# ultralytics/yolov3

Hardware: AMD Instinct MI355X
Metric: images/sec (640x640) inference+NMS (higher is better)
Workload: dtype f16; 1 GPU; yolov3 inference 640x640 batch=32/GPU fp16 nc=80 + NMS(conf 0.001, iou 0.6, multi_label, max_det 300) [BASELINE configs[1]]; global_batch=32, parallelism=replicas x1 (no data-path collective)

## Files before the change

### yolov3_amd/csrc/api.cpp

```cpp
#include <atomic>
#include <mutex>
#include <stdarg.h>
#include <stdio.h>
#include <stdlib.h>
#include <string.h>

#include "../../include/yolov3_hip.h"
#include "y3_knobs.h"

static thread_local char g_err[512] = "";

void y3_set_error(const char* fmt, ...) {
    va_list ap;
    va_start(ap, fmt);
    vsnprintf(g_err, sizeof(g_err), fmt, ap);
    va_end(ap);
}

extern "C" const char* y3_last_error(void) { return g_err; }
extern "C" int y3_abi_version(void) { return Y3_ABI_VERSION; }

namespace {
struct Knob {
    const char* name;
    long long def;
};
const Knob kKnobs[] = {
    {"conv", 0}, {"conv_ahead", 3}, {"bn_nt_bytes", 64ll << 20},
    {"wgrad", 0}, {"wgrad_xcd", 2}, {"dgrad_quad", 1}, {"spp_direct", 0}, {"wgrad_strip", 1}, {"conv_strip", 1},
    {"conv_v10", 1}, {"v10_mp", 0}, {"v10_blocks", 0}, {"v10_half", 2}, {"v10_ksplit", 1}, {"v10_slices", 0},
    {"v10_group", 1}, {"tile_xcd", 1}, {"conv_1x1s", 1}, {"wgrad_patch", 1}, {"wgrad_blocks", 512}, {"nms_sort", 1},
    {"decode_tile", 1},
};
constexpr int kCount = (int)(sizeof(kKnobs) / sizeof(kKnobs[0]));
static_assert(kCount == Y3K_COUNT, "kKnobs and y3_knob_id (y3_common.h) list the same knobs in the same order");
std::atomic<long long> g_val[kCount];
std::once_flag g_once;

int knob_index(const char* key) {
    for (int i = 0; i < kCount; ++i)
        if (key && !strcmp(key, kKnobs[i].name)) return i;
    return -1;
}
void load_defaults() {
    for (int i = 0; i < kCount; ++i) g_val[i].store(kKnobs[i].def, std::memory_order_relaxed);
    const char* e = getenv("Y3_TUNE");
    if (!e) return;
    char buf[512];
    strncpy(buf, e, sizeof(buf) - 1);
    buf[sizeof(buf) - 1] = 0;
    for (char* tok = strtok(buf, ",;"); tok; tok = strtok(nullptr, ",;")) {
        char* eq = strchr(tok, '=');
        if (!eq) continue;
        *eq = 0;
        const int i = knob_index(tok);
        if (i >= 0) g_val[i].store(atoll(eq + 1), std::memory_order_relaxed);
        else fprintf(stderr, "libyolov3_hip: Y3_TUNE names an unknown knob '%s'\n", tok);
    }
}
}

long long y3_knob(int id) {
    std::call_once(g_once, load_defaults);
    return (id >= 0 && id < kCount) ? g_val[id].load(std::memory_order_relaxed) : 0;
}
// ... 27 lines not shown
```

### yolov3_amd/csrc/detect_nms.hip

```cpp
#include "y3_common.h"

#include <rocprim/rocprim.hpp>

#include <atomic>

namespace {

template <typename T>
Y3_DEV float decode_one(float v, int o, int x, int y, float stride, float aw, float ah);

template <typename T>
__global__ __launch_bounds__(256) void decode_kernel(const T* __restrict__ head, int bs, int ny, int nx, int pitch, int na, int no, float aw0, float ah0,
                                                       float aw1, float ah1, float aw2, float ah2, float aw3, float ah3, float aw4, float ah4, float stride,
                                                       T* __restrict__ raw, T* __restrict__ z, long long row_offset, long long total_rows) {
    const int nch = na * no;
    const long long idx = (long long)blockIdx.x * 256 + threadIdx.x;
    const long long total = (long long)bs * ny * nx * nch;
    if (idx >= total) return;
    const int ch = (int)(idx % nch);
    long long t = idx / nch;
    const int x = (int)(t % nx);
    t /= nx;
    const int y = (int)(t % ny);
    const int b = (int)(t / ny);
// ... 185 lines not shown
            if (want_z) *(vec8*)((T*)job.z + (it.b * zimg + (L.row_offset + (long long)it.p0) * no) + off) = zv;
        }
    };
    const int step = gridDim.x;
    int item = blockIdx.x;
    Item ic = locate(item), i0, i1 = locate(item + step);
    uint4 v0 = load(ic), v1 = load(i1);
    ((uint4*)stage[0])[tid] = v0;
    __syncthreads();
    while (item < job.items) {
        i0 = locate(item + 2 * step);
        v0 = load(i0);
        compute(ic, stage[0], stage[1], v1);
        __syncthreads();
        ic = i1;
        if ((item += step) >= job.items) break;
        i1 = locate(item + 2 * step);
        v1 = load(i1);
        compute(ic, stage[1], stage[0], v0);
        __syncthreads();
        ic = i0;
        item += step;
    }
}

constexpr int IMG_BITS = 11, ORD_BITS = 21, CLS_BITS = 12, RANK_BITS = 15;
constexpr unsigned long long KEY_UNUSED = ~0ull;

struct NmsWs {
    int* row_count;
    int* row_off;
    unsigned* img_maxabs;
    unsigned* img_total;
    unsigned long long* key_a;
    unsigned long long* key_b;
    unsigned* val_a;
    unsigned* val_b;
    unsigned long long* key_c;
    unsigned* val_c;
    float4* cbox;
    float* cscore;
    int* ccls;
    float4* sbox;
    unsigned char* keep;
    void* tmp;
    size_t tmp_bytes;
    long long cap;
    int own_sort;
};

template <typename T> Y3_DEV bool gt_thr(float v, float thr_T) { return v > thr_T; }

Y3_DEV bool class_allowed(int c, const int* __restrict__ classes, int ncf) {
    if (ncf == 0) return true;
    bool ok = false;
    for (int i = 0; i < ncf; ++i) ok |= (classes[i] == c);
    return ok;
}

constexpr int NMS_ROW_BATCH = 8;
template <typename T, int MODE>
__global__ __launch_bounds__(256) void nms_candidates_kernel(const T* __restrict__ pred, int bs, int n_rows, int nc, float thr, int multi_label,
                                                               const int* __restrict__ classes, int ncf, NmsWs ws, int* __restrict__ status, int ord_shift) {
    const int lane = threadIdx.x & 63;
    const int chunks_per_img = (n_rows + 63) / 64;
    const long long wave_id = (long long)blockIdx.x * 4 + (threadIdx.x >> 6);
// ... 140 lines not shown
            cnt = ok ? 1 : 0;
            if (MODE == 1 && ok && lane == 0) {
                const long long g = off;
                if (g < ws.cap) {
                    const unsigned ord = (unsigned)((g - img_off0) >> ord_shift);
                    ws.cbox[g] = box;
                    ws.cscore[g] = best;
                    ws.ccls[g] = bi;
                    if (!ws.own_sort) {
                        ws.key_a[g] = ((unsigned long long)img << (32 + ORD_BITS)) | ((unsigned long long)(~__float_as_uint(best)) << ORD_BITS) |
                                      (unsigned long long)(ord & ((1u << ORD_BITS) - 1u));
                        ws.val_a[g] = (unsigned)g;
                    }
                } else {
                    status[0] = 1;
                }
            }
        }
        if (MODE == 1 && cnt > 0) {
            const float m4 = fmaxf(fmaxf(fabsf(box.x), fabsf(box.y)), fmaxf(fabsf(box.z), fabsf(box.w)));
            maxabs = (m4 == m4) ? fmaxf(maxabs, m4) : INFINITY;
        }
        if (lane == r) mycount = cnt;
    }
    if (MODE == 0) {
        if (myrow < n_rows) ws.row_count[(long long)img * n_rows + myrow] = mycount;
        if (ws.own_sort) {
            int t = mycount;
#pragma unroll
            for (int d = 32; d >= 1; d >>= 1) t += __shfl_xor(t, d);
            if (lane == 0 && t > 0) atomicAdd(&ws.img_total[img * 64 + (int)(wave_id & 63)], (unsigned)t);
        }
    } else {
        if (lane == 0 && maxabs > 0.0f) atomicMax(&ws.img_maxabs[img], __float_as_uint(maxabs));
    }
}

constexpr int SCAN_PER = 33, SCAN_CHUNK = 1024 * SCAN_PER;
__global__ __launch_bounds__(1024) void nms_scan_kernel(NmsWs ws, int bs, int n_rows) {
    __shared__ unsigned buf[SCAN_CHUNK];
    __shared__ unsigned wsum[16];
    const int img = blockIdx.x, tid = threadIdx.x, lane = tid & 63, wv = tid >> 6;
    auto block_sum_scan = [&](unsigned v, unsigned& excl, unsigned& total) {
        unsigned inc = v;
#pragma unroll
        for (int d = 1; d < 64; d <<= 1) {
            const unsigned o = __shfl_up(inc, d);
            if (lane >= d) inc += o;
        }
        __syncthreads();
        if (lane == 63) wsum[wv] = inc;
        __syncthreads();
        unsigned before = 0, all = 0;
#pragma unroll
        for (int w = 0; w < 16; ++w) {
            const unsigned t = wsum[w];
            if (w < wv) before += t;
            all += t;
        }
        excl = before + inc - v;
        total = all;
    };
    unsigned prev = 0;
    for (int j = tid; j < img * 64; j += 1024) prev += ws.img_total[j];
    unsigned e0, carry;
    block_sum_scan(prev, e0, carry);
    const int* __restrict__ cnt = ws.row_count + (long long)img * n_rows;
    int* __restrict__ off = ws.row_off + (long long)img * n_rows;
// ... 7 lines not shown
        for (int r = r0; r < r1; ++r) mine += buf[r];
        unsigned excl, total;
        block_sum_scan(mine, excl, total);
        unsigned run = carry + excl;
        for (int r = r0; r < r1; ++r) {
            const unsigned c = buf[r];
            buf[r] = run;
            run += c;
        }
        __syncthreads();
        for (int i = tid; i < n; i += 1024) off[c0 + i] = (int)buf[i];
        carry += total;
    }
    if (img == bs - 1 && tid == 0) ws.row_off[(long long)bs * n_rows] = (int)carry;
}

__global__ __launch_bounds__(256) void nms_rank_kernel(NmsWs ws, int bs, int n_rows, int max_nms, float max_wh, int agnostic, const unsigned long long* __restrict__ key1,
                                                        const unsigned* __restrict__ idx1, unsigned long long* __restrict__ key2, unsigned* __restrict__ val2,
                                                        int* __restrict__ status) {
    const long long i = (long long)blockIdx.x * 256 + threadIdx.x;
    if (i >= ws.cap) return;
    const long long total = ws.row_off[(long long)bs * n_rows];
    if (i == 0) status[1] = (int)(total > 0x7fffffffLL ? 0x7fffffff : total);
    unsigned long long k2 = KEY_UNUSED;
    ws.keep[i] = 0;
    if (i < total && key1[i] != KEY_UNUSED) {
        const int img = (int)(key1[i] >> (32 + ORD_BITS));
        const long long start = ws.row_off[(long long)img * n_rows];
        const long long rank = i - start;
        if (rank < max_nms) {
            const unsigned g = idx1[i];
            const int cls = ws.ccls[g];
            const float4 b = ws.cbox[g];
            const bool part = !agnostic && (__uint_as_float(ws.img_maxabs[img]) < max_wh * 0.5f);
            const float c = (float)cls * (agnostic ? 0.0f : max_wh);
            ws.sbox[i] = make_float4(b.x + c, b.y + c, b.z + c, b.w + c);
            const unsigned seg = part ? (unsigned)cls : 0u;
            k2 = ((unsigned long long)img << (CLS_BITS + RANK_BITS)) | ((unsigned long long)seg << RANK_BITS) | (unsigned long long)rank;
        }
    }
    key2[i] = k2;
    val2[i] = (unsigned)i;
}

constexpr int SORT_WAVES = 16, SORT_NB = 512;
struct SortLds {
    unsigned hist[SORT_WAVES * SORT_NB];
    unsigned tot[SORT_NB];
};
Y3_DEV unsigned ld_l2(const unsigned* p) { return __hip_atomic_load(p, __ATOMIC_RELAXED, __HIP_MEMORY_SCOPE_AGENT); }

template <typename Load, typename Digit, typename Put>
Y3_DEV void counting_pass(SortLds& L, const int cnt, const int bits, Load load, Digit digit, Put put) {
    const int tid = threadIdx.x, lane = tid & 63, wv = tid >> 6;
    const int nb = 1 << bits;
    for (int i = tid; i < SORT_WAVES * nb; i += SORT_WAVES * 64) L.hist[(i >> bits) * SORT_NB + (i & (nb - 1))] = 0u;
    __syncthreads();
    const int per = (((cnt + SORT_WAVES - 1) / SORT_WAVES) + 63) & ~63;
    const int lo = wv * per, hi = cnt < lo + per ? cnt : lo + per;
    for (int c0 = lo; c0 < hi; c0 += 256) {
        uint2 e[4];
#pragma unroll
        for (int u = 0; u < 4; ++u) {
            const int r = c0 + 64 * u + lane;
            e[u] = load(r < hi ? r : lo);
        }
#pragma unroll
        for (int u = 0; u < 4; ++u) {
            const int r = c0 + 64 * u + lane;
            if (r < hi) atomicAdd(&L.hist[wv * SORT_NB + digit(e[u].x)], 1u);
        }
    }
    __syncthreads();
    if (tid < nb) {
        unsigned run = 0;
#pragma unroll
        for (int w = 0; w < SORT_WAVES; ++w) {
            const unsigned t = L.hist[w * SORT_NB + tid];
            L.hist[w * SORT_NB + tid] = run;
            run += t;
        }
        L.tot[tid] = run;
    }
    __syncthreads();
    if (wv == 0) {
        unsigned v[SORT_NB / 64], sum = 0;
#pragma unroll
        for (int k = 0; k < SORT_NB / 64; ++k) {
            const int d = lane * (SORT_NB / 64) + k;
            v[k] = d < nb ? L.tot[d] : 0u;
            sum += v[k];
        }
        unsigned inc = sum;
#pragma unroll
        for (int d = 1; d < 64; d <<= 1) {
            const unsigned o = __shfl_up(inc, d);
            if (lane >= d) inc += o;
        }
        unsigned run = inc - sum;
#pragma unroll
        for (int k = 0; k < SORT_NB / 64; ++k) {
            const int d = lane * (SORT_NB / 64) + k;
            if (d < nb) L.tot[d] = run;
            run += v[k];
        }
    }
    __syncthreads();
    volatile unsigned* H = L.hist + wv * SORT_NB;
    const unsigned long long below = (1ull << lane) - 1ull;
    for (int c0 = lo; c0 < hi; c0 += 256) {
        uint2 e[4];
#pragma unroll
        for (int u = 0; u < 4; ++u) {
            const int r = c0 + 64 * u + lane;
            e[u] = load(r < hi ? r : lo);
        }
#pragma unroll
        for (int u = 0; u < 4; ++u) {
            if (c0 + 64 * u >= hi) break;
            const int r = c0 + 64 * u + lane;
            const bool valid = r < hi;
            const unsigned d = digit(e[u].x);
            unsigned long long peers = __ballot(valid);
            for (int b = 0; b < bits; ++b) {
                const bool bit = (d >> b) & 1u;
                const unsigned long long m = __ballot(valid && bit);
                peers &= bit ? m : ~m;
            }
            if (valid) {
                const unsigned base = H[d];
                put(L.tot[d] + base + (unsigned)__builtin_popcountll(peers & below), e[u].x, e[u].y);
                if ((peers >> lane) == 1ull) H[d] = base + (unsigned)__builtin_popcountll(peers);
            }
        }
    }
    __syncthreads();
}

__global__ __launch_bounds__(SORT_WAVES * 64) void nms_sort_kernel(NmsWs ws, int bs, int n_rows, int max_nms, float max_wh, int agnostic, int nseg, int sbit0, int sbits,
                                                                     int n_sp, int* __restrict__ status) {
    __shared__ SortLds L;
    const int img = blockIdx.x, tid = threadIdx.x;
    const long long total = ws.row_off[(long long)bs * n_rows];
    if (img == 0 && tid == 0) status[1] = (int)(total > 0x7fffffffLL ? 0x7fffffff : total);
    const long long start = ws.row_off[(long long)img * n_rows];
    long long cnt_ll = (long long)ws.row_off[(long long)(img + 1) * n_rows] - start;
    if (start + cnt_ll > ws.cap) cnt_ll = ws.cap - start > 0 ? ws.cap - start : 0;
    const int cnt = (int)cnt_ll;
    if (cnt <= 0) return;
    unsigned* const X0 = (unsigned*)ws.key_a + start, * const X1 = (unsigned*)ws.key_a + ws.cap + start;
    unsigned* const X2 = (unsigned*)ws.key_b + start, * const X3 = (unsigned*)ws.key_b + ws.cap + start;
    unsigned* const X4 = (unsigned*)ws.key_c + start, * const X5 = (unsigned*)ws.key_c + ws.cap + start;
    unsigned* const VA = ws.val_a + start, * const VB = ws.val_b + start, * const VC = ws.val_c + start;
    const float* __restrict__ score = ws.cscore + start;

    const unsigned dmask = (1u << sbits) - 1u;
    for (int p = 0; p < n_sp; ++p) {
        const int shift = sbit0 + p * sbits;
        const bool last = p == n_sp - 1;
        const unsigned* kin = p == 1 ? X0 : p == 2 ? X2 : X5;
        const unsigned* vin = p == 1 ? X1 : p == 2 ? X3 : VA;
        unsigned* kout = p == 0 ? X0 : p == 1 ? X2 : X5;
        unsigned* vout = last ? VB : p == 0 ? X1 : p == 1 ? X3 : VA;
        counting_pass(
            L, cnt, sbits,
            [&](int r) { return p == 0 ? make_uint2(~__float_as_uint(score[r]), (unsigned)(start + r)) : make_uint2(ld_l2(kin + r), ld_l2(vin + r)); },
            [&](unsigned k) { return (k >> shift) & dmask; },
            [&](unsigned pos, unsigned k, unsigned v) {
                if (!last) kout[pos] = k;
                vout[pos] = v;
            });
    }

    const int cntm = cnt < max_nms ? cnt : max_nms;
    const bool part = !agnostic && nseg > 1 && (__uint_as_float(ws.img_maxabs[img]) < max_wh * 0.5f);
    for (int r = tid; r < cntm; r += SORT_WAVES * 64) {
        const unsigned g = ld_l2(VB + r);
        const float4 b = ws.cbox[g];
        const float c = (float)ws.ccls[g] * (agnostic ? 0.0f : max_wh);
        ws.sbox[start + r] = make_float4(b.x + c, b.y + c, b.z + c, b.w + c);
        ws.keep[start + r] = 0;
        if (!part) { VC[r] = (unsigned)(start + r); X4[r] = 0u; }
    }
    if (!part) return;
    int cbits = 1;
    while ((1 << cbits) < nseg) ++cbits;
    auto seg_of = [&](int r) { return make_uint2((unsigned)ws.ccls[ld_l2(VB + r)], (unsigned)(start + r)); };
    if (cbits <= 9) {
        counting_pass(L, cntm, cbits, seg_of, [&](unsigned k) { return k; }, [&](unsigned pos, unsigned k, unsigned v) { X4[pos] = k; VC[pos] = v; });
    } else {
        counting_pass(L, cntm, 9, seg_of, [&](unsigned k) { return k & 511u; }, [&](unsigned pos, unsigned k, unsigned v) { X0[pos] = k; X1[pos] = v; });
        counting_pass(
            L, cntm, cbits - 9, [&](int r) { return make_uint2(ld_l2(X0 + r), ld_l2(X1 + r)); }, [&](unsigned k) { return k >> 9; },
            [&](unsigned pos, unsigned k, unsigned v) { X4[pos] = k; VC[pos] = v; });
    }
}

Y3_DEV long long lower_bound_u64(const unsigned long long* __restrict__ a, long long n, unsigned long long v) {
    long long lo = 0, hi = n;
    while (lo < hi) {
        const long long mid = (lo + hi) >> 1;
        if (a[mid] < v) lo = mid + 1; else hi = mid;
    }
    return lo;
}

Y3_DEV long long lower_bound_u32(const unsigned* __restrict__ a, long long n, unsigned v) {
    long long lo = 0, hi = n;
    while (lo < hi) {
        const long long mid = (lo + hi) >> 1;
        if (a[mid] < v) lo = mid + 1; else hi = mid;
    }
    return lo;
}

__global__ __launch_bounds__(256) void nms_greedy_kernel(NmsWs ws, int nseg, double iou_thr, int max_det, int max_nms, const unsigned long long* __restrict__ key2,
                                                          const unsigned* __restrict__ pos2, const unsigned* __restrict__ seg_sorted, int n_rows) {
    __shared__ unsigned removed[(1 << RANK_BITS) / 32];
    __shared__ float4 blk[64];
    __shared__ unsigned long long srow[64];
    __shared__ unsigned long long s_keepm;
    __shared__ int s_kept;
    const int img = blockIdx.x / nseg, seg = blockIdx.x % nseg;
    long long lo, hi;
    if (seg_sorted) {
        const long long start = ws.row_off[(long long)img * n_rows];
        long long cnt = (long long)ws.row_off[(long long)(img + 1) * n_rows] - start;
        if (start + cnt > ws.cap) cnt = ws.cap - start > 0 ? ws.cap - start : 0;
        if (cnt > max_nms) cnt = max_nms;
        lo = start + lower_bound_u32(seg_sorted + start, cnt, (unsigned)seg);
        hi = start + lower_bound_u32(seg_sorted + start, cnt, (unsigned)seg + 1u);
    } else {
        const unsigned long long kbase = ((unsigned long long)img << (CLS_BITS + RANK_BITS)) | ((unsigned long long)seg << RANK_BITS);
        lo = lower_bound_u64(key2, ws.cap, kbase);
        hi = lower_bound_u64(key2, ws.cap, kbase + (1ull << RANK_BITS));
    }
    const int n = (int)(hi - lo);
    if (n <= 0) return;
    const int tid = threadIdx.x, lane = tid & 63, wv = tid >> 6;
    for (int w = tid; w < 2 * ((n + 63) / 64); w += 256) removed[w] = 0u;
    if (tid == 0) s_kept = 0;
    const unsigned* __restrict__ pos = pos2 + lo;
    auto suppresses = [&](const float4 bi, const float iarea, const float4 bj) {
        const float xx1 = fmaxf(bi.x, bj.x), yy1 = fmaxf(bi.y, bj.y);
        const float xx2 = fminf(bi.z, bj.z), yy2 = fminf(bi.w, bj.w);
        float w = xx2 - xx1, h = yy2 - yy1;
        w = w > 0.0f ? w : 0.0f;
        h = h > 0.0f ? h : 0.0f;
        const float inter = w * h;
        const float jarea = (bj.z - bj.x) * (bj.w - bj.y);
        const float ovr = inter / (iarea + jarea - inter);
        return (double)ovr > iou_thr;
    };
    for (int base = 0; base < n; base += 64) {
        const int cnt = n - base < 64 ? n - base : 64;
        __syncthreads();
        const unsigned long long rem_in = (unsigned long long)removed[base >> 5] | ((unsigned long long)removed[(base >> 5) + 1] << 32);
        const unsigned long long valid = cnt == 64 ? ~0ull : ((1ull << cnt) - 1ull);
        if ((rem_in & valid) == valid) continue;
        if (tid < 64) {
            if (tid < cnt) blk[tid] = ws.sbox[pos[base + tid]];
            srow[tid] = 0ull;
// ... 12 lines not shown
        }
        __syncthreads();
        if (wv == 0) {
            const unsigned long long row = srow[lane];
            const int row_lo = (int)(unsigned)row, row_hi = (int)(unsigned)(row >> 32);
            unsigned long long rem = rem_in, keepm = 0ull;
            int kept = s_kept;
            for (int i = 0; i < cnt && kept < max_det; ++i) {
                if (!((rem >> i) & 1ull)) {
                    keepm |= 1ull << i;
                    ++kept;
                    rem |= (unsigned long long)(unsigned)__builtin_amdgcn_readlane(row_lo, i) | ((unsigned long long)(unsigned)__builtin_amdgcn_readlane(row_hi, i) << 32);
                }
            }
            if ((keepm >> lane) & 1ull) ws.keep[pos[base + lane]] = 1;
            if (lane == 0) { s_keepm = keepm; s_kept = kept; }
        }
        __syncthreads();
        const unsigned long long keepm = s_keepm;
        if (s_kept >= max_det) break;
        if (keepm)
            for (int j = base + 64 + tid; j < n; j += 256) {
                if (removed[j >> 5] & (1u << (j & 31))) continue;
                const float4 bj = ws.sbox[pos[j]];
                unsigned long long km = keepm;
                while (km) {
                    const int i = __builtin_ctzll(km);
                    km &= km - 1ull;
                    const float4 bi = blk[i];
                    if (suppresses(bi, (bi.z - bi.x) * (bi.w - bi.y), bj)) { atomicOr(&removed[j >> 5], 1u << (j & 31)); break; }
                }
            }
    }
}

__global__ __launch_bounds__(256) void nms_gather_kernel(NmsWs ws, int n_rows, int max_det, int max_nms, const unsigned* __restrict__ idx1,
                                                          float* __restrict__ out_rows, int* __restrict__ out_counts) {
    __shared__ int wave_cnt[4];
    __shared__ int s_base;
    const int img = blockIdx.x;
    const long long start = ws.row_off[(long long)img * n_rows];
    long long cnt = (long long)ws.row_off[(long long)(img + 1) * n_rows] - start;
    if (start + cnt > ws.cap) cnt = ws.cap - start > 0 ? ws.cap - start : 0;
    if (cnt > max_nms) cnt = max_nms;
    const int tid = threadIdx.x, lane = tid & 63, wv = tid >> 6;
    if (tid == 0) s_base = 0;
    __syncthreads();
    for (long long c0 = 0; c0 < cnt; c0 += 256) {
        const long long i = c0 + tid;
        const bool k = (i < cnt) && ws.keep[start + i];
        const unsigned long long m = __ballot(k);
        if (lane == 0) wave_cnt[wv] = __builtin_popcountll(m);
        __syncthreads();
        int before = s_base;
        for (int w = 0; w < wv; ++w) before += wave_cnt[w];
        const int slot = before + __builtin_popcountll(m & ((1ull << lane) - 1ull));
        if (k && slot < max_det) {
            const unsigned g = idx1[start + i];
            const float4 b = ws.cbox[g];
            float* o = out_rows + ((long long)img * max_det + slot) * 6;
            o[0] = b.x; o[1] = b.y; o[2] = b.z; o[3] = b.w;
            o[4] = ws.cscore[g];
            o[5] = (float)ws.ccls[g];
        }
        __syncthreads();
        if (tid == 0) s_base += wave_cnt[0] + wave_cnt[1] + wave_cnt[2] + wave_cnt[3];
        __syncthreads();
        if (s_base >= max_det) break;
    }
    if (tid == 0) out_counts[img] = s_base < max_det ? s_base : max_det;
}

size_t align_up(size_t v) { return (v + 255) & ~(size_t)255; }

long long worst_capacity(int bs, int n_rows, int nc, const y3_nms_params* p) {
    return (long long)bs * n_rows * ((p->multi_label && nc > 1) ? nc : 1);
}
long long default_capacity(int bs, int n_rows, int nc, const y3_nms_params* p) {
    const long long worst = worst_capacity(bs, n_rows, nc, p);
    long long cap = (long long)bs * 16384;
    if (cap > worst) cap = worst;
    if (cap < 1024) cap = 1024;
    return cap;
}

size_t temp_bytes(long long cap, size_t scan_n) {
    size_t a = 0, b = 0;
    (void)rocprim::radix_sort_pairs(nullptr, a, (unsigned long long*)nullptr, (unsigned long long*)nullptr, (unsigned*)nullptr, (unsigned*)nullptr, (size_t)cap, 0u,
                                    64u, (hipStream_t)0);
    (void)rocprim::exclusive_scan(nullptr, b, (int*)nullptr, (int*)nullptr, 0, scan_n + 1, rocprim::plus<int>(), (hipStream_t)0);
    return align_up(a > b ? a : b);
}

size_t carve(NmsWs& ws, unsigned char* base, int bs, long long cap, size_t scan_n) {
    size_t off = 0;
    auto take = [&](size_t bytes) {
        unsigned char* p = base ? base + off : nullptr;
        off += align_up(bytes);
        return p;
    };
    ws.cap = cap;
    ws.row_count = (int*)take((scan_n + 1) * sizeof(int));
    ws.row_off = (int*)take((scan_n + 1) * sizeof(int));
    ws.img_maxabs = (unsigned*)take((size_t)65 * bs * sizeof(unsigned));
    ws.img_total = ws.img_maxabs ? ws.img_maxabs + bs : nullptr;
    ws.key_a = (unsigned long long*)take((size_t)cap * 8);
    ws.key_b = (unsigned long long*)take((size_t)cap * 8);
    ws.key_c = (unsigned long long*)take((size_t)cap * 8);
    ws.val_a = (unsigned*)take((size_t)cap * 4);
    ws.val_b = (unsigned*)take((size_t)cap * 4);
    ws.val_c = (unsigned*)take((size_t)cap * 4);
    ws.cbox = (float4*)take((size_t)cap * 16);
    ws.cscore = (float*)take((size_t)cap * 4);
    ws.ccls = (int*)take((size_t)cap * 4);
    ws.sbox = (float4*)take((size_t)cap * 16);
    ws.keep = (unsigned char*)take((size_t)cap);
    ws.tmp_bytes = temp_bytes(cap, scan_n);
    ws.tmp = take(ws.tmp_bytes);
    return off;
}

template <typename T>
int run_nms(const void* pred, int bs, int n_rows, int nc, const y3_nms_params* p, const int* classes, float* out_rows, int* out_counts, int* out_status,
            long long capacity, void* workspace, size_t workspace_bytes, hipStream_t st) {
    const size_t scan_n = (size_t)bs * n_rows;
    long long cap = capacity > 0 ? capacity : default_capacity(bs, n_rows, nc, p);
    const long long worst = worst_capacity(bs, n_rows, nc, p);
    if (cap > worst) cap = worst;
    if (cap < 1024) cap = 1024;
    NmsWs ws;
    const size_t need = carve(ws, nullptr, bs, cap, scan_n);
    if (need > workspace_bytes) Y3_FAIL("y3_nms: workspace too small (%zu bytes given, %zu needed for capacity %lld)", workspace_bytes, need, cap);
    if (cap > 0x7ffffff0LL) Y3_FAIL("y3_nms: capacity too large");
    carve(ws, (unsigned char*)workspace, bs, cap, scan_n);

    const float thr = (float)(T)(p->conf_thres);
    const int multi = (p->multi_label && nc > 1) ? 1 : 0;
    const int ncf = classes ? p->n_classes_filter : 0;
    int ord_shift = 0;
    while ((((long long)n_rows * (multi ? nc : 1)) >> ord_shift) >= (1ll << ORD_BITS)) ++ord_shift;
    const bool one_seg = p->agnostic != 0;
    const int nseg = one_seg ? 1 : nc;

    Y3_HIP(hipMemsetAsync(out_status, 0, 2 * sizeof(int), st));
    Y3_HIP(hipMemsetAsync(ws.img_maxabs, 0, (size_t)65 * bs * sizeof(unsigned), st));
    ws.own_sort = y3_knob(Y3K_NMS_SORT) != 0 ? 1 : 0;
    if (!ws.own_sort) Y3_HIP(hipMemsetAsync(ws.key_a, 0xff, (size_t)cap * 8, st));
    Y3_HIP(hipMemsetAsync(ws.row_count + scan_n, 0, sizeof(int), st));

    const long long waves = (long long)bs * ((n_rows + 63) / 64);
    const unsigned cblocks = (unsigned)((waves + 3) / 4);
    hipLaunchKernelGGL((nms_candidates_kernel<T, 0>), dim3(cblocks), dim3(256), 0, st, (const T*)pred, bs, n_rows, nc, thr, multi, classes, ncf, ws, out_status, ord_shift);
    Y3_CHECK_LAUNCH();
    size_t tb = ws.tmp_bytes;
    if (ws.own_sort) {
        hipLaunchKernelGGL(nms_scan_kernel, dim3((unsigned)bs), dim3(1024), 0, st, ws, bs, n_rows);
        Y3_CHECK_LAUNCH();
    } else if (rocprim::exclusive_scan(ws.tmp, tb, ws.row_count, ws.row_off, 0, scan_n + 1, rocprim::plus<int>(), st) != hipSuccess) Y3_FAIL("y3_nms: scan failed");
    hipLaunchKernelGGL((nms_candidates_kernel<T, 1>), dim3(cblocks), dim3(256), 0, st, (const T*)pred, bs, n_rows, nc, thr, multi, classes, ncf, ws, out_status, ord_shift);
    Y3_CHECK_LAUNCH();
    if (ws.own_sort) {
        const bool narrow = sizeof(T) == 2;
        hipLaunchKernelGGL(nms_sort_kernel, dim3((unsigned)bs), dim3(SORT_WAVES * 64), 0, st, ws, bs, n_rows, p->max_nms, p->max_wh, p->agnostic, nseg, narrow ? 13 : 0,
                           narrow ? 9 : 8, narrow ? 2 : 4, out_status);
        Y3_CHECK_LAUNCH();
        hipLaunchKernelGGL(nms_greedy_kernel, dim3((unsigned)(bs * nseg)), dim3(256), 0, st, ws, nseg, p->iou_thres, p->max_det, p->max_nms,
                           (const unsigned long long*)nullptr, ws.val_c, (const unsigned*)ws.key_c, n_rows);
        Y3_CHECK_LAUNCH();
        hipLaunchKernelGGL(nms_gather_kernel, dim3((unsigned)bs), dim3(256), 0, st, ws, n_rows, p->max_det, p->max_nms, ws.val_b, out_rows, out_counts);
        Y3_CHECK_LAUNCH();
        return 0;
    }
    tb = ws.tmp_bytes;
    if (rocprim::radix_sort_pairs(ws.tmp, tb, ws.key_a, ws.key_b, ws.val_a, ws.val_b, (size_t)cap, 0u, 64u, st) != hipSuccess) Y3_FAIL("y3_nms: sort-1 failed");
    const unsigned rblocks = (unsigned)((cap + 255) / 256);
    hipLaunchKernelGGL(nms_rank_kernel, dim3(rblocks), dim3(256), 0, st, ws, bs, n_rows, p->max_nms, p->max_wh, p->agnostic, ws.key_b, ws.val_b, ws.key_a, ws.val_a,
                       out_status);
    Y3_CHECK_LAUNCH();
    tb = ws.tmp_bytes;
    if (rocprim::radix_sort_pairs(ws.tmp, tb, ws.key_a, ws.key_c, ws.val_a, ws.val_c, (size_t)cap, 0u, (unsigned)(IMG_BITS + CLS_BITS + RANK_BITS), st) != hipSuccess)
        Y3_FAIL("y3_nms: sort-2 failed");
    hipLaunchKernelGGL(nms_greedy_kernel, dim3((unsigned)(bs * nseg)), dim3(256), 0, st, ws, nseg, p->iou_thres, p->max_det, p->max_nms, ws.key_c, ws.val_c,
                       (const unsigned*)nullptr, n_rows);
    Y3_CHECK_LAUNCH();
    hipLaunchKernelGGL(nms_gather_kernel, dim3((unsigned)bs), dim3(256), 0, st, ws, n_rows, p->max_det, p->max_nms, ws.val_b, out_rows, out_counts);
    Y3_CHECK_LAUNCH();
    return 0;
}

}

extern "C" size_t y3_nms_workspace_bytes(int32_t bs, int32_t n_rows, int32_t nc, const y3_nms_params* p, int64_t capacity) {
    if (!p || bs <= 0 || n_rows <= 0 || nc <= 0) return 0;
    long long cap = capacity > 0 ? capacity : default_capacity(bs, n_rows, nc, p);
    const long long worst = worst_capacity(bs, n_rows, nc, p);
    if (cap > worst) cap = worst;
    if (cap < 1024) cap = 1024;
    NmsWs ws;
    return carve(ws, nullptr, bs, cap, (size_t)bs * n_rows);
}

extern "C" int y3_nms(const void* pred, int32_t dtype, int32_t bs, int32_t n_rows, int32_t nc, const y3_nms_params* p, const int32_t* classes, float* out_rows,
                      int32_t* out_counts, int32_t* out_status, int64_t capacity, void* workspace, size_t workspace_bytes, void* stream) {
    if (!pred || !p || !out_rows || !out_counts || !out_status || !workspace) Y3_FAIL("y3_nms: null argument");
    if (!(p->conf_thres >= 0.0f && p->conf_thres <= 1.0f)) Y3_FAIL("Invalid Confidence threshold %g, valid values are between 0.0 and 1.0", (double)p->conf_thres);
    if (!(p->iou_thres >= 0.0 && p->iou_thres <= 1.0)) Y3_FAIL("Invalid IoU %g, valid values are between 0.0 and 1.0", p->iou_thres);
    if (bs <= 0 || bs >= (1 << IMG_BITS) - 1) Y3_FAIL("y3_nms: batch size %d unsupported (max %d)", bs, (1 << IMG_BITS) - 2);
    if (nc <= 0 || nc >= (1 << CLS_BITS)) Y3_FAIL("y3_nms: class count %d unsupported", nc);
    if (p->max_nms <= 0 || p->max_nms > (1 << RANK_BITS) - 1) Y3_FAIL("y3_nms: max_nms %d unsupported (max %d)", p->max_nms, (1 << RANK_BITS) - 1);
    if ((long long)bs * n_rows >= 0x7fffffffLL) Y3_FAIL("y3_nms: too many rows");
    if (p->max_det <= 0) Y3_FAIL("y3_nms: max_det must be positive");
    hipStream_t st = (hipStream_t)stream;
    switch (dtype) {
        case Y3_F16: return run_nms<f16_t>(pred, bs, n_rows, nc, p, classes, out_rows, out_counts, out_status, capacity, workspace, workspace_bytes, st);
        case Y3_BF16: return run_nms<bf16_t>(pred, bs, n_rows, nc, p, classes, out_rows, out_counts, out_status, capacity, workspace, workspace_bytes, st);
        case Y3_F32: return run_nms<float>(pred, bs, n_rows, nc, p, classes, out_rows, out_counts, out_status, capacity, workspace, workspace_bytes, st);
    }
    Y3_FAIL("y3_nms: bad dtype %d", dtype);
// ... 156 lines not shown
```

### yolov3_amd/csrc/y3_knobs.h

```cpp
#pragma once
enum y3_knob_id {
    Y3K_CONV = 0,
    Y3K_CONV_AHEAD,
    Y3K_BN_NT_BYTES,
    Y3K_WGRAD,
    Y3K_WGRAD_XCD,
    Y3K_DGRAD_QUAD,
    Y3K_SPP_DIRECT,
    Y3K_WGRAD_STRIP,
    Y3K_CONV_STRIP,
    Y3K_CONV_V10,
    Y3K_V10_MP,
    Y3K_V10_BLOCKS,
    Y3K_V10_HALF,
    Y3K_V10_KSPLIT,
    Y3K_V10_SLICES,
    Y3K_V10_GROUP,
    Y3K_TILE_XCD,
    Y3K_CONV_1X1S,
    Y3K_WGRAD_PATCH,
    Y3K_WGRAD_BLOCKS,
    Y3K_NMS_SORT,
    Y3K_DECODE_TILE,
    Y3K_COUNT
};
long long y3_knob(int id);
```

### yolov3_amd/ops.py

```python
from __future__ import annotations

import ctypes as C
from dataclasses import dataclass
from typing import NamedTuple

import math

import torch

from . import _lib
from ._lib import Y3AugmentItem, Y3AugmentMosaic, Y3AugmentTile, Y3ConvDesc, Y3DatasetImage, Y3NmsParams, Y3Tensor, check

DTYPE_CODE = {torch.float16: _lib.Y3_F16, torch.bfloat16: _lib.Y3_BF16, torch.float32: _lib.Y3_F32, torch.uint8: _lib.Y3_U8}


def dtype_code(dt: torch.dtype) -> int:
    try:
        return DTYPE_CODE[dt]
    except KeyError:
        raise TypeError(f"dtype {dt} is not supported by the MI355X path (float16 / bfloat16 / float32)") from None


def require_gpu(t: torch.Tensor, what: str):
    if not t.is_cuda:
# ... 378 lines not shown

_nms_ws_cache: dict = {}


def nms_raw(pred: torch.Tensor, conf_thres: float, iou_thres: float, classes, agnostic: bool, multi_label: bool, max_det: int, max_nms: int = 30000,
            max_wh: float = 7680.0):
    require_gpu(pred, "non_max_suppression")
    pred = pred.contiguous()
    bs, n_rows, no = pred.shape
    nc = no - 5
    dev = pred.device
    cls_t = torch.tensor(list(classes), dtype=torch.int32, device=dev) if classes is not None else None
    p = Y3NmsParams(float(iou_thres), float(conf_thres), int(bool(multi_label)), int(bool(agnostic)), int(max_det), int(max_nms), float(max_wh),
                    0 if cls_t is None else cls_t.numel())
    L = _lib.lib()
    rows = torch.empty(bs, max_det, 6, dtype=torch.float32, device=dev)
    meta = torch.empty(bs + 2, dtype=torch.int32, device=dev)
    capacity = 0
    for attempt in range(3):
        need = int(L.y3_nms_workspace_bytes(bs, n_rows, nc, C.byref(p), capacity))
        key = (dev.index, need)
        ws = _nms_ws_cache.get(key)
        if ws is None:
            ws = torch.empty(need, dtype=torch.uint8, device=dev)
            if need <= (1 << 30):
                _nms_ws_cache[key] = ws
        check(
            L.y3_nms(pred.data_ptr(), dtype_code(pred.dtype), bs, n_rows, nc, C.byref(p), cls_t.data_ptr() if cls_t is not None else None, rows.data_ptr(),
                     meta.data_ptr(), meta.data_ptr() + bs * 4, capacity, ws.data_ptr(), need, stream_ptr()),
            "y3_nms",
        )
        m = meta.tolist()
        nms_raw.last_candidates = m[bs + 1]
        if m[bs] == 0:
            return rows, m[:bs]
        capacity = max(m[bs + 1], 1)
    raise _lib.Y3Error("y3_nms: candidate capacity overflow persisted")


def scale_boxes_raw(rows: torch.Tensor, img_stride: int, row_stride: int, counts: torch.Tensor | None, bs: int, max_rows: int, params: torch.Tensor):
    require_gpu(rows, "scale_boxes")
    check(_lib.lib().y3_scale_boxes(rows.data_ptr(), int(img_stride), int(row_stride), counts.data_ptr() if counts is not None else None, int(bs), int(max_rows),
                                    params.data_ptr(), stream_ptr()), "y3_scale_boxes")


def match_detections_raw(dets: torch.Tensor, img_stride: int, row_stride: int, counts: torch.Tensor | None, bs: int, max_det: int, labels: torch.Tensor,
                         offsets: torch.Tensor, iouv: torch.Tensor) -> torch.Tensor:
    require_gpu(dets, "process_batch")
    correct = torch.empty(bs, max_det, iouv.numel(), dtype=torch.uint8, device=dets.device)
    check(_lib.lib().y3_match_detections(dets.data_ptr(), int(img_stride), int(row_stride), counts.data_ptr() if counts is not None else None, int(bs), int(max_det),
                                         labels.data_ptr() if labels.numel() else None, offsets.data_ptr(), iouv.data_ptr(), int(iouv.numel()), correct.data_ptr(), stream_ptr()),
          "y3_match_detections")
    return correct


def val_stats_append(conf: torch.Tensor, cls: torch.Tensor, img_stride: int, elem_stride: int, counts: torch.Tensor | None, bs: int, max_det: int, correct: torch.Tensor,
                     dst_conf: torch.Tensor, dst_cls: torch.Tensor, dst_mask: torch.Tensor, dst_offset: int):
    require_gpu(conf, "ValStats")
    require_gpu(correct, "ValStats")
    if conf.dtype != torch.float32 or cls.dtype != torch.float32 or correct.dtype not in (torch.uint8, torch.bool) or not correct.is_contiguous():
        raise TypeError("val_stats_append expects fp32 confidences / classes and a contiguous uint8 / bool (rows, T) hit matrix")
    check(_lib.lib().y3_val_stats_append(conf.data_ptr(), cls.data_ptr(), int(img_stride), int(elem_stride), counts.data_ptr() if counts is not None else None, int(bs), int(max_det),
                                         correct.data_ptr(), int(correct.shape[-1]), dst_conf.data_ptr(), dst_cls.data_ptr(), dst_mask.data_ptr(), int(dst_offset),
                                         int(dst_conf.numel()), stream_ptr()), "y3_val_stats_append")


def val_stats_count_labels(cls: torch.Tensor, stride: int, n: int, nt: torch.Tensor):
# ... 621 lines not shown
```

Before: 5224 images/sec.

## Add two-round head-limited NMS that sorts only top-scoring candidates first

Adds an nms_head knob, defaulting to 1216, that makes the own-sort NMS path run in two rounds. Round one finds a radix cutoff from a score histogram and sorts only the top-scoring head. It then runs greedy NMS on that head and counts kept boxes per image. Round two redoes the full sort and greedy pass only for images that kept fewer than max_det boxes and had candidates beyond the head. The per-image maxabs reduction is also spread over 64 slots to cut atomic contention, and the status word now encodes round-2 counts. It adds extra histogram passes and relaunches, and it risks duplicated work when many images need the second round.

```diff
diff --git a/yolov3_amd/csrc/api.cpp b/yolov3_amd/csrc/api.cpp
--- a/yolov3_amd/csrc/api.cpp
+++ b/yolov3_amd/csrc/api.cpp
@@ -30,7 +30,7 @@
     {"wgrad", 0}, {"wgrad_xcd", 2}, {"dgrad_quad", 1}, {"spp_direct", 0}, {"wgrad_strip", 1}, {"conv_strip", 1},
     {"conv_v10", 1}, {"v10_mp", 0}, {"v10_blocks", 0}, {"v10_half", 2}, {"v10_ksplit", 1}, {"v10_slices", 0},
     {"v10_group", 1}, {"tile_xcd", 1}, {"conv_1x1s", 1}, {"wgrad_patch", 1}, {"wgrad_blocks", 512}, {"nms_sort", 1},
-    {"decode_tile", 1},
+    {"decode_tile", 1}, {"nms_head", 1216},
 };
 constexpr int kCount = (int)(sizeof(kKnobs) / sizeof(kKnobs[0]));
 static_assert(kCount == Y3K_COUNT, "kKnobs and y3_knob_id (y3_common.h) list the same knobs in the same order");
diff --git a/yolov3_amd/csrc/detect_nms.hip b/yolov3_amd/csrc/detect_nms.hip
--- a/yolov3_amd/csrc/detect_nms.hip
+++ b/yolov3_amd/csrc/detect_nms.hip
@@ -241,6 +241,8 @@
     int* row_off;
     unsigned* img_maxabs;
     unsigned* img_total;
+    unsigned* img_head;
+    unsigned* img_kept;
     unsigned long long* key_a;
     unsigned long long* key_b;
     unsigned* val_a;
@@ -447,8 +449,18 @@
             if (lane == 0 && t > 0) atomicAdd(&ws.img_total[img * 64 + (int)(wave_id & 63)], (unsigned)t);
         }
     } else {
-        if (lane == 0 && maxabs > 0.0f) atomicMax(&ws.img_maxabs[img], __float_as_uint(maxabs));
-    }
+        if (lane == 0 && maxabs > 0.0f) atomicMax(&ws.img_maxabs[img * 64 + (int)(wave_id & 63)], __float_as_uint(maxabs));
+    }
+}
+
+Y3_DEV float img_max_coord(const NmsWs& ws, int img) {
+    unsigned m = ws.img_maxabs[img * 64 + (threadIdx.x & 63)];
+#pragma unroll
+    for (int d = 32; d >= 1; d >>= 1) {
+        const unsigned o = __shfl_xor(m, d);
+        m = o > m ? o : m;
+    }
+    return __uint_as_float(m);
 }
 
 constexpr int SCAN_PER = 33, SCAN_CHUNK = 1024 * SCAN_PER;
@@ -522,7 +534,9 @@
             const unsigned g = idx1[i];
             const int cls = ws.ccls[g];
             const float4 b = ws.cbox[g];
-            const bool part = !agnostic && (__uint_as_float(ws.img_maxabs[img]) < max_wh * 0.5f);
+            unsigned mx = 0u;
+            for (int s = 0; s < 64; ++s) mx = ws.img_maxabs[img * 64 + s] > mx ? ws.img_maxabs[img * 64 + s] : mx;
+            const bool part = !agnostic && (__uint_as_float(mx) < max_wh * 0.5f);
             const float c = (float)cls * (agnostic ? 0.0f : max_wh);
             ws.sbox[i] = make_float4(b.x + c, b.y + c, b.z + c, b.w + c);
             const unsigned seg = part ? (unsigned)cls : 0u;
@@ -537,11 +551,12 @@
 struct SortLds {
     unsigned hist[SORT_WAVES * SORT_NB];
     unsigned tot[SORT_NB];
+    unsigned cut[3];
 };
 Y3_DEV unsigned ld_l2(const unsigned* p) { return __hip_atomic_load(p, __ATOMIC_RELAXED, __HIP_MEMORY_SCOPE_AGENT); }
 
-template <typename Load, typename Digit, typename Put>
-Y3_DEV void counting_pass(SortLds& L, const int cnt, const int bits, Load load, Digit digit, Put put) {
+template <typename Load, typename Digit, typename Put, typename Member>
+Y3_DEV void counting_pass(SortLds& L, const int cnt, const int bits, Load load, Digit digit, Put put, Member member) {
     const int tid = threadIdx.x, lane = tid & 63, wv = tid >> 6;
     const int nb = 1 << bits;
     for (int i = tid; i < SORT_WAVES * nb; i += SORT_WAVES * 64) L.hist[(i >> bits) * SORT_NB + (i & (nb - 1))] = 0u;
@@ -558,7 +573,7 @@
 #pragma unroll
         for (int u = 0; u < 4; ++u) {
             const int r = c0 + 64 * u + lane;
-            if (r < hi) atomicAdd(&L.hist[wv * SORT_NB + digit(e[u].x)], 1u);
+            if (r < hi && member(e[u].x)) atomicAdd(&L.hist[wv * SORT_NB + digit(e[u].x)], 1u);
         }
     }
     __syncthreads();
@@ -609,7 +624,7 @@
         for (int u = 0; u < 4; ++u) {
             if (c0 + 64 * u >= hi) break;
             const int r = c0 + 64 * u + lane;
-            const bool valid = r < hi;
+            const bool valid = r < hi && member(e[u].x);
             const unsigned d = digit(e[u].x);
             unsigned long long peers = __ballot(valid);
             for (int b = 0; b < bits; ++b) {
@@ -626,18 +641,73 @@
     }
     __syncthreads();
 }
+template <typename Load, typename Digit, typename Put>
+Y3_DEV void counting_pass(SortLds& L, const int cnt, const int bits, Load load, Digit digit, Put put) {
+    counting_pass(L, cnt, bits, load, digit, put, [](unsigned) { return true; });
+}
+
+template <typename Load, typename Digit, typename Member>
+Y3_DEV void head_cutoff(SortLds& L, const int cnt, const int bits, const unsigned want, Load load, Digit digit, Member member) {
+    const int tid = threadIdx.x, lane = tid & 63;
+    const int nb = 1 << bits;
+    for (int i = tid; i < nb; i += SORT_WAVES * 64) L.tot[i] = 0u;
+    __syncthreads();
+    for (int c0 = 0; c0 < cnt; c0 += SORT_WAVES * 64 * 4) {
+        uint2 e[4];
+#pragma unroll
+        for (int u = 0; u < 4; ++u) {
+            const int r = c0 + SORT_WAVES * 64 * u + tid;
+            e[u] = load(r < cnt ? r : 0);
+        }
+#pragma unroll
+        for (int u = 0; u < 4; ++u)
+            if (c0 + SORT_WAVES * 64 * u + tid < cnt && member(e[u].x)) atomicAdd(&L.tot[digit(e[u].x)], 1u);
+    }
+    __syncthreads();
+    if (tid < 64) {
+        unsigned v[SORT_NB / 64], sum = 0;
+#pragma unroll
+        for (int k = 0; k < SORT_NB / 64; ++k) {
+            const int d = lane * (SORT_NB / 64) + k;
+            v[k] = d < nb ? L.tot[d] : 0u;
+            sum += v[k];
+        }
+        unsigned inc = sum;
+#pragma unroll
+        for (int d = 1; d < 64; d <<= 1) {
+            const unsigned o = __shfl_up(inc, d);
+            if (lane >= d) inc += o;
+        }
+        unsigned run = inc - sum;
+#pragma unroll
+        for (int k = 0; k < SORT_NB / 64; ++k) {
+            if (run < want && run + v[k] >= want) {
+                L.cut[0] = (unsigned)(lane * (SORT_NB / 64) + k);
+                L.cut[1] = run + v[k];
+                L.cut[2] = run;
+            }
+            run += v[k];
+        }
+    }
+    __syncthreads();
+}
 
 __global__ __launch_bounds__(SORT_WAVES * 64) void nms_sort_kernel(NmsWs ws, int bs, int n_rows, int max_nms, float max_wh, int agnostic, int nseg, int sbit0, int sbits,
-                                                                     int n_sp, int* __restrict__ status) {
+                                                                     int n_sp, int head, int round, int max_det, int* __restrict__ status) {
     __shared__ SortLds L;
     const int img = blockIdx.x, tid = threadIdx.x;
     const long long total = ws.row_off[(long long)bs * n_rows];
-    if (img == 0 && tid == 0) status[1] = (int)(total > 0x7fffffffLL ? 0x7fffffff : total);
+    if (img == 0 && tid == 0 && round < 2) status[1] = (int)(total > 0x7fffffffLL ? 0x7fffffff : total);
     const long long start = ws.row_off[(long long)img * n_rows];
     long long cnt_ll = (long long)ws.row_off[(long long)(img + 1) * n_rows] - start;
     if (start + cnt_ll > ws.cap) cnt_ll = ws.cap - start > 0 ? ws.cap - start : 0;
     const int cnt = (int)cnt_ll;
     if (cnt <= 0) return;
+    const int cntm = cnt < max_nms ? cnt : max_nms;
+    if (round == 2) {
+        if (ws.img_kept[img] >= (unsigned)max_det || (int)ws.img_head[img] == cntm) return;
+        if (tid == 0) atomicAdd(&status[0], 2);
+    }
     unsigned* const X0 = (unsigned*)ws.key_a + start, * const X1 = (unsigned*)ws.key_a + ws.cap + start;
     unsigned* const X2 = (unsigned*)ws.key_b + start, * const X3 = (unsigned*)ws.key_b + ws.cap + start;
     unsigned* const X4 = (unsigned*)ws.key_c + start, * const X5 = (unsigned*)ws.key_c + ws.cap + start;
@@ -645,6 +715,24 @@
     const float* __restrict__ score = ws.cscore + start;
 
     const unsigned dmask = (1u << sbits) - 1u;
+    const int top = sbit0 + (n_sp - 1) * sbits;
+    auto fresh = [&](int r) { return make_uint2(~__float_as_uint(score[r]), (unsigned)(start + r)); };
+    unsigned cut1 = dmask, cut2 = dmask;
+    int ns = cnt;
+    auto top_of = [&](unsigned k) { return (k >> top) & dmask; };
+    auto next_of = [&](unsigned k) { return (k >> (top - sbits)) & dmask; };
+    if (round == 1 && head > 0 && cnt > head) {
+        head_cutoff(L, cnt, sbits, (unsigned)head, fresh, top_of, [](unsigned) { return true; });
+        cut1 = L.cut[0];
+        const unsigned below = L.cut[2];
+        head_cutoff(L, cnt, sbits, (unsigned)head - below, fresh, next_of, [&](unsigned k) { return top_of(k) == cut1; });
+        cut2 = L.cut[0];
+        ns = (int)(below + L.cut[1]);
+    }
+    auto in_head = [&](unsigned k) {
+        const unsigned t = top_of(k);
+        return t < cut1 || (t == cut1 && next_of(k) <= cut2);
+    };
     for (int p = 0; p < n_sp; ++p) {
         const int shift = sbit0 + p * sbits;
         const bool last = p == n_sp - 1;
@@ -653,18 +741,23 @@
         unsigned* kout = p == 0 ? X0 : p == 1 ? X2 : X5;
         unsigned* vout = last ? VB : p == 0 ? X1 : p == 1 ? X3 : VA;
         counting_pass(
-            L, cnt, sbits,
-            [&](int r) { return p == 0 ? make_uint2(~__float_as_uint(score[r]), (unsigned)(start + r)) : make_uint2(ld_l2(kin + r), ld_l2(vin + r)); },
+            L, p == 0 ? cnt : ns, sbits, [&](int r) { return p == 0 ? fresh(r) : make_uint2(ld_l2(kin + r), ld_l2(vin + r)); },
             [&](unsigned k) { return (k >> shift) & dmask; },
             [&](unsigned pos, unsigned k, unsigned v) {
                 if (!last) kout[pos] = k;
                 vout[pos] = v;
-            });
-    }
-
-    const int cntm = cnt < max_nms ? cnt : max_nms;
-    const bool part = !agnostic && nseg > 1 && (__uint_as_float(ws.img_maxabs[img]) < max_wh * 0.5f);
-    for (int r = tid; r < cntm; r += SORT_WAVES * 64) {
+            },
+            in_head);
+    }
+
+    int prep = ns < max_nms ? ns : max_nms;
+    if (round == 1) {
+        const int h = head < 0 ? -head : head;
+        if (prep > h) prep = h;
+        if (tid == 0) ws.img_head[img] = (unsigned)prep;
+    }
+    const bool part = !agnostic && nseg > 1 && (img_max_coord(ws, img) < max_wh * 0.5f);
+    for (int r = tid; r < prep; r += SORT_WAVES * 64) {
         const unsigned g = ld_l2(VB + r);
         const float4 b = ws.cbox[g];
         const float c = (float)ws.ccls[g] * (agnostic ? 0.0f : max_wh);
@@ -677,11 +770,11 @@
     while ((1 << cbits) < nseg) ++cbits;
     auto seg_of = [&](int r) { return make_uint2((unsigned)ws.ccls[ld_l2(VB + r)], (unsigned)(start + r)); };
     if (cbits <= 9) {
-        counting_pass(L, cntm, cbits, seg_of, [&](unsigned k) { return k; }, [&](unsigned pos, unsigned k, unsigned v) { X4[pos] = k; VC[pos] = v; });
+        counting_pass(L, prep, cbits, seg_of, [&](unsigned k) { return k; }, [&](unsigned pos, unsigned k, unsigned v) { X4[pos] = k; VC[pos] = v; });
     } else {
-        counting_pass(L, cntm, 9, seg_of, [&](unsigned k) { return k & 511u; }, [&](unsigned pos, unsigned k, unsigned v) { X0[pos] = k; X1[pos] = v; });
+        counting_pass(L, prep, 9, seg_of, [&](unsigned k) { return k & 511u; }, [&](unsigned pos, unsigned k, unsigned v) { X0[pos] = k; X1[pos] = v; });
         counting_pass(
-            L, cntm, cbits - 9, [&](int r) { return make_uint2(ld_l2(X0 + r), ld_l2(X1 + r)); }, [&](unsigned k) { return k >> 9; },
+            L, prep, cbits - 9, [&](int r) { return make_uint2(ld_l2(X0 + r), ld_l2(X1 + r)); }, [&](unsigned k) { return k >> 9; },
             [&](unsigned pos, unsigned k, unsigned v) { X4[pos] = k; VC[pos] = v; });
     }
 }
@@ -705,7 +798,7 @@
 }
 
 __global__ __launch_bounds__(256) void nms_greedy_kernel(NmsWs ws, int nseg, double iou_thr, int max_det, int max_nms, const unsigned long long* __restrict__ key2,
-                                                          const unsigned* __restrict__ pos2, const unsigned* __restrict__ seg_sorted, int n_rows) {
+                                                          const unsigned* __restrict__ pos2, const unsigned* __restrict__ seg_sorted, int n_rows, int round) {
     __shared__ unsigned removed[(1 << RANK_BITS) / 32];
     __shared__ float4 blk[64];
     __shared__ unsigned long long srow[64];
@@ -718,6 +811,8 @@
         long long cnt = (long long)ws.row_off[(long long)(img + 1) * n_rows] - start;
         if (start + cnt > ws.cap) cnt = ws.cap - start > 0 ? ws.cap - start : 0;
         if (cnt > max_nms) cnt = max_nms;
+        if (round == 1) cnt = ws.img_head[img];
+        else if (round == 2 && (ws.img_kept[img] >= (unsigned)max_det || (long long)ws.img_head[img] == cnt)) return;
         lo = start + lower_bound_u32(seg_sorted + start, cnt, (unsigned)seg);
         hi = start + lower_bound_u32(seg_sorted + start, cnt, (unsigned)seg + 1u);
     } else {
@@ -796,10 +891,11 @@
                 }
             }
     }
+    if (round == 1 && tid == 0 && s_kept > 0) atomicAdd(&ws.img_kept[img], (unsigned)s_kept);
 }
 
 __global__ __launch_bounds__(256) void nms_gather_kernel(NmsWs ws, int n_rows, int max_det, int max_nms, const unsigned* __restrict__ idx1,
-                                                          float* __restrict__ out_rows, int* __restrict__ out_counts) {
+                                                          float* __restrict__ out_rows, int* __restrict__ out_counts, int rounds) {
     __shared__ int wave_cnt[4];
     __shared__ int s_base;
     const int img = blockIdx.x;
@@ -807,6 +903,7 @@
     long long cnt = (long long)ws.row_off[(long long)(img + 1) * n_rows] - start;
     if (start + cnt > ws.cap) cnt = ws.cap - start > 0 ? ws.cap - start : 0;
     if (cnt > max_nms) cnt = max_nms;
+    if (rounds == 2 && ws.img_kept[img] >= (unsigned)max_det) cnt = ws.img_head[img];
     const int tid = threadIdx.x, lane = tid & 63, wv = tid >> 6;
     if (tid == 0) s_base = 0;
     __syncthreads();
@@ -856,6 +953,8 @@
     return align_up(a > b ? a : b);
 }
 
+size_t ctrl_words(int bs) { return 1 + (size_t)(64 + 64 + 1 + 1) * bs; }
+
 size_t carve(NmsWs& ws, unsigned char* base, int bs, long long cap, size_t scan_n) {
     size_t off = 0;
     auto take = [&](size_t bytes) {
@@ -864,10 +963,12 @@
         return p;
     };
     ws.cap = cap;
-    ws.row_count = (int*)take((scan_n + 1) * sizeof(int));
+    ws.row_count = (int*)take((scan_n + ctrl_words(bs)) * sizeof(int));
+    ws.img_maxabs = ws.row_count ? (unsigned*)ws.row_count + scan_n + 1 : nullptr;
+    ws.img_total = ws.img_maxabs ? ws.img_maxabs + (size_t)64 * bs : nullptr;
+    ws.img_head = ws.img_maxabs ? ws.img_total + (size_t)64 * bs : nullptr;
+    ws.img_kept = ws.img_maxabs ? ws.img_head + bs : nullptr;
     ws.row_off = (int*)take((scan_n + 1) * sizeof(int));
-    ws.img_maxabs = (unsigned*)take((size_t)65 * bs * sizeof(unsigned));
-    ws.img_total = ws.img_maxabs ? ws.img_maxabs + bs : nullptr;
     ws.key_a = (unsigned long long*)take((size_t)cap * 8);
     ws.key_b = (unsigned long long*)take((size_t)cap * 8);
     ws.key_c = (unsigned long long*)take((size_t)cap * 8);
@@ -907,10 +1008,9 @@
     const int nseg = one_seg ? 1 : nc;
 
     Y3_HIP(hipMemsetAsync(out_status, 0, 2 * sizeof(int), st));
-    Y3_HIP(hipMemsetAsync(ws.img_maxabs, 0, (size_t)65 * bs * sizeof(unsigned), st));
+    Y3_HIP(hipMemsetAsync(ws.row_count + scan_n, 0, ctrl_words(bs) * sizeof(int), st));
     ws.own_sort = y3_knob(Y3K_NMS_SORT) != 0 ? 1 : 0;
     if (!ws.own_sort) Y3_HIP(hipMemsetAsync(ws.key_a, 0xff, (size_t)cap * 8, st));
-    Y3_HIP(hipMemsetAsync(ws.row_count + scan_n, 0, sizeof(int), st));
 
     const long long waves = (long long)bs * ((n_rows + 63) / 64);
     const unsigned cblocks = (unsigned)((waves + 3) / 4);
@@ -925,13 +1025,19 @@
     Y3_CHECK_LAUNCH();
     if (ws.own_sort) {
         const bool narrow = sizeof(T) == 2;
-        hipLaunchKernelGGL(nms_sort_kernel, dim3((unsigned)bs), dim3(SORT_WAVES * 64), 0, st, ws, bs, n_rows, p->max_nms, p->max_wh, p->agnostic, nseg, narrow ? 13 : 0,
-                           narrow ? 9 : 8, narrow ? 2 : 4, out_status);
-        Y3_CHECK_LAUNCH();
-        hipLaunchKernelGGL(nms_greedy_kernel, dim3((unsigned)(bs * nseg)), dim3(256), 0, st, ws, nseg, p->iou_thres, p->max_det, p->max_nms,
-                           (const unsigned long long*)nullptr, ws.val_c, (const unsigned*)ws.key_c, n_rows);
-        Y3_CHECK_LAUNCH();
-        hipLaunchKernelGGL(nms_gather_kernel, dim3((unsigned)bs), dim3(256), 0, st, ws, n_rows, p->max_det, p->max_nms, ws.val_b, out_rows, out_counts);
+        long long head = y3_knob(Y3K_NMS_HEAD);
+        if (head > (1 << RANK_BITS)) head = 1 << RANK_BITS;
+        if (head < -(1 << RANK_BITS)) head = -(1 << RANK_BITS);
+        const int rounds = head != 0 ? 2 : 1;
+        for (int r = rounds == 2 ? 1 : 0; r <= (rounds == 2 ? 2 : 0); ++r) {
+            hipLaunchKernelGGL(nms_sort_kernel, dim3((unsigned)bs), dim3(SORT_WAVES * 64), 0, st, ws, bs, n_rows, p->max_nms, p->max_wh, p->agnostic, nseg,
+                               narrow ? 13 : 0, narrow ? 9 : 8, narrow ? 2 : 4, (int)head, r, p->max_det, out_status);
+            Y3_CHECK_LAUNCH();
+            hipLaunchKernelGGL(nms_greedy_kernel, dim3((unsigned)(bs * nseg)), dim3(256), 0, st, ws, nseg, p->iou_thres, p->max_det, p->max_nms,
+                               (const unsigned long long*)nullptr, ws.val_c, (const unsigned*)ws.key_c, n_rows, r);
+            Y3_CHECK_LAUNCH();
+        }
+        hipLaunchKernelGGL(nms_gather_kernel, dim3((unsigned)bs), dim3(256), 0, st, ws, n_rows, p->max_det, p->max_nms, ws.val_b, out_rows, out_counts, rounds);
         Y3_CHECK_LAUNCH();
         return 0;
     }
@@ -945,9 +1051,9 @@
     if (rocprim::radix_sort_pairs(ws.tmp, tb, ws.key_a, ws.key_c, ws.val_a, ws.val_c, (size_t)cap, 0u, (unsigned)(IMG_BITS + CLS_BITS + RANK_BITS), st) != hipSuccess)
         Y3_FAIL("y3_nms: sort-2 failed");
     hipLaunchKernelGGL(nms_greedy_kernel, dim3((unsigned)(bs * nseg)), dim3(256), 0, st, ws, nseg, p->iou_thres, p->max_det, p->max_nms, ws.key_c, ws.val_c,
-                       (const unsigned*)nullptr, n_rows);
+                       (const unsigned*)nullptr, n_rows, 0);
     Y3_CHECK_LAUNCH();
-    hipLaunchKernelGGL(nms_gather_kernel, dim3((unsigned)bs), dim3(256), 0, st, ws, n_rows, p->max_det, p->max_nms, ws.val_b, out_rows, out_counts);
+    hipLaunchKernelGGL(nms_gather_kernel, dim3((unsigned)bs), dim3(256), 0, st, ws, n_rows, p->max_det, p->max_nms, ws.val_b, out_rows, out_counts, 1);
     Y3_CHECK_LAUNCH();
     return 0;
 }
diff --git a/yolov3_amd/csrc/y3_knobs.h b/yolov3_amd/csrc/y3_knobs.h
--- a/yolov3_amd/csrc/y3_knobs.h
+++ b/yolov3_amd/csrc/y3_knobs.h
@@ -22,6 +22,7 @@
     Y3K_WGRAD_BLOCKS,
     Y3K_NMS_SORT,
     Y3K_DECODE_TILE,
+    Y3K_NMS_HEAD,
     Y3K_COUNT
 };
 long long y3_knob(int id);
diff --git a/yolov3_amd/ops.py b/yolov3_amd/ops.py
--- a/yolov3_amd/ops.py
+++ b/yolov3_amd/ops.py
@@ -434,7 +434,8 @@
         )
         m = meta.tolist()
         nms_raw.last_candidates = m[bs + 1]
-        if m[bs] == 0:
+        nms_raw.last_round2 = m[bs] >> 1
+        if (m[bs] & 1) == 0:
             return rows, m[:bs]
         capacity = max(m[bs + 1], 1)
     raise _lib.Y3Error("y3_nms: candidate capacity overflow persisted")
```

Result: faster. 5331 images/sec, median of 6 (+2.0%).
